# george-tyler-315-incline/ggml-neon-opt

Hardware: AMD Instinct MI355X
Metric: tg128 tok/s + Q4_K GEMV achieved-HBM-GB/s, TinyLlama-1.1B Q4_K_M @1 GPU (higher is better)
Workload: dtype q4_K/q6_K x q8_K (u4/u6*i8 dot4 -> i32, f32 combine); 1 GPU; tinyllama-1.1b Q4_K_M tg2221: full decode graph, token i at position i of a fresh f16 KV cache; parallelism=replicas x1, hipgraph=True

## Files before the change

### ggml-neon-opt_amd/csrc/kq_rows.hip

```cpp
#include <hip/hip_ext.h>

#include "kq_internal.h"
#include "kq_ops_device.h"
#include "kq_rows_device.h"

#ifndef KQ_ROWS_DIAG
#define KQ_ROWS_DIAG 0
#endif
#if KQ_ROWS_DIAG
#define RDIAG(ld) ((ld).diag)
#define RSTAMPS(h) ((h).stamps)
#define RSTAMP() __builtin_amdgcn_s_memrealtime()
#else
#define RDIAG(ld) 0
#define RSTAMPS(h) ((uint64_t *)nullptr)
#define RSTAMP() ((uint64_t)0)
#endif

#ifndef KQ_ROWS_XMODE
#define KQ_ROWS_XMODE 0
#endif
#ifndef KQ_ROWS_PRE0
#define KQ_ROWS_PRE0 1
#endif
#ifndef KQ_ROWS_L2PF
#define KQ_ROWS_L2PF 0
#endif
#ifndef KQ_ROWS_MASKED
#define KQ_ROWS_MASKED 2
#endif
#ifndef KQ_ROWS_LINT_BREAK
#define KQ_ROWS_LINT_BREAK 0
#endif

#ifndef KQ_ROWS_PRIO
#define KQ_ROWS_PRIO 0
#endif

#ifndef KQ_ROWS_YSC1
#define KQ_ROWS_YSC1 1
#endif

namespace kq {

__device__ __forceinline__ void store_y(float *p, float v) {
    if (KQ_ROWS_YSC1) asm volatile("global_store_dword %0, %1, off sc1" ::"v"(p), "v"(v) : "memory");
    else *p = v;
}

template <bool AM>
__global__ void __launch_bounds__(WG_THREADS) kq_quantize_q8L(const float *__restrict__ x, int64_t x_stride,
                                                              uint8_t *__restrict__ y, int nb, int64_t nblocks) {
    const int lane = threadIdx.x & 63;
    const int64_t bi = (int64_t)blockIdx.x * 16 + (threadIdx.x >> 4);
    if (bi >= nblocks) return;
    const int64_t row = bi / nb;
    const int b = (int)(bi - row * nb);
    const float *xb = x + row * x_stride + (int64_t)b * QK + 16 * (lane & 15);
    u32x4 v[4];
#pragma unroll
    for (int k = 0; k < 4; ++k) v[k] = *(const u32x4 *)(xb + 4 * k);
    quant16_store<AM>(v, lane & 15, y + bi * Q8L_STRIDE);
}
template __global__ void kq_quantize_q8L<false>(const float *, int64_t, uint8_t *, int, int64_t);
template __global__ void kq_quantize_q8L<true>(const float *, int64_t, uint8_t *, int, int64_t);

__global__ void __launch_bounds__(256) kq_rms_norm_q8L(const float *__restrict__ x, const float *__restrict__ w,
                                                       uint8_t *__restrict__ yq, int64_t n, float eps) {
    extern __shared__ __attribute__((aligned(16))) double sb_sum[];
    const int64_t row = blockIdx.x;
    const float *xr = x + row * n;
    const int nb = (int)(n / QK);
    const int rid = threadIdx.x >> 4, l = threadIdx.x & 15;
    for (int b0 = 0; b0 < nb; b0 += 16) {
        const int b = b0 + rid;
        double s = 0.0;
        if (b < nb) {
            float v[16];
            const float4 *p = (const float4 *)(xr + (int64_t)b * QK + 16 * l);
#pragma unroll
            for (int k = 0; k < 4; ++k) {
                const float4 t = p[k];
                v[4 * k] = t.x, v[4 * k + 1] = t.y, v[4 * k + 2] = t.z, v[4 * k + 3] = t.w;
            }
            s = sumsq16(v);
        }
        s = row16_sum(s);
        if (b < nb && l == 0) sb_sum[b] = s;
    }
    __syncthreads();
    double total = seq_sum_lds(sb_sum, nb);
    if (rms_mean_ambiguous(div_by_count(total, n), n)) {
        __syncthreads();
        if (threadIdx.x < 64) {
            const double s = seq_sumsq_wave(xr, n, threadIdx.x);
            if (threadIdx.x == 0) sb_sum[0] = s;
        }
        __syncthreads();
        total = sb_sum[0];
    }
    const float mean = (float)div_by_count(total, n);
    const float scale = 1.0f / sqrtf(mean + eps);
    for (int b0 = 0; b0 < nb; b0 += 16) {
        const int b = b0 + rid;
        if (b >= nb) continue;
        const float4 *p = (const float4 *)(xr + (int64_t)b * QK + 16 * l);
        const float4 *q = (const float4 *)(w + (int64_t)b * QK + 16 * l);
        u32x4 v[4];
#pragma unroll
        for (int k = 0; k < 4; ++k) {
            const float4 t = p[k], m = q[k];
            v[k].x = __float_as_uint((t.x * scale) * m.x);
// ... 187 lines not shown
template <int LSH>
struct RowsPrologue {
    static constexpr int NP = LSH ? 1 : ROWS_QPASS;
    static constexpr int NL = 4 >> LSH;
    static constexpr int LP = 16 << LSH;
    static constexpr int SPW = 4 >> LSH;
    u32x4 xv[NP][NL];
    u32x4 x2v[NP][NL];
    int qw = 0;
    int nb, pass, rot, wave, lane;

    __device__ __forceinline__ int slot(int i) const { return pass * i + SPW * wave + (lane >> (4 + LSH)); }
    __device__ __forceinline__ int sl() const { return lane & (LP - 1); }
    __device__ __forceinline__ int sbk(int j) const {
        const int b = (j < nb ? j : nb - 1) + rot;
        return b >= nb ? b - nb : b;
    }

    template <int PRO, bool ASM = true>
    __device__ __forceinline__ void load(const RowsLead &ld, int wave_, int lane_, int rot_, int diag) {
        nb = ld.nb, pass = SPW * ld.nwv, rot = rot_, wave = wave_, lane = lane_;
        const float *const x = (const float *)ld.x;
        const float *const x2 = (diag & 16) ? x : ld.x2;
#pragma unroll
        for (int i = 0; i < NP; ++i) qw += (i < ld.qiters && pass * i + SPW * wave < nb) ? 1 : 0;
#pragma unroll
        for (int i = 0; i < NP; ++i)
#pragma unroll
            for (int k = 0; k < NL; ++k) {
                asm volatile("" : "=v"(xv[i][k]));
                if (PRO != ROWS_PRO_NONE) asm volatile("" : "=v"(x2v[i][k]));
            }
#pragma unroll
        for (int i = 0; i < NP; ++i) {
            if (i < qw) {
                const int64_t e = (int64_t)sbk(slot(i)) * QK + (16 >> LSH) * sl();
#pragma unroll
                for (int k = 0; k < NL; ++k) {
                    if (ASM) gload16_into(xv[i][k], x + e + 4 * k);
                    else xv[i][k] = *(const u32x4 *)(x + e + 4 * k);
                }
                if (PRO != ROWS_PRO_NONE) {
#pragma unroll
                    for (int k = 0; k < NL; ++k) {
                        if (ASM) gload16_into(x2v[i][k], x2 + e + 4 * k);
                        else x2v[i][k] = *(const u32x4 *)(x2 + e + 4 * k);
                    }
                }
            }
        }
    }

    template <int PRO>
    __device__ __forceinline__ void pin() {
        if constexpr (LSH == 0) {
            asm volatile("" : "+v"(xv[0][0]), "+v"(xv[0][1]), "+v"(xv[0][2]), "+v"(xv[0][3]), "+v"(xv[1][0]),
                         "+v"(xv[1][1]), "+v"(xv[1][2]), "+v"(xv[1][3]), "+v"(xv[2][0]), "+v"(xv[2][1]),
                         "+v"(xv[2][2]), "+v"(xv[2][3]));
        } else {
#pragma unroll
            for (int k = 0; k < NL; ++k) asm volatile("" : "+v"(xv[0][k]));
        }
        if (PRO != ROWS_PRO_NONE) {
#pragma unroll
            for (int i = 0; i < NP; ++i)
#pragma unroll
                for (int k = 0; k < NL; ++k) asm volatile("" : "+v"(x2v[i][k]));
        }
    }

    __device__ __forceinline__ void swiglu_pass(int i) {
#pragma unroll
        for (int k = 0; k < NL; ++k) xv[i][k] = swiglu4(xv[i][k], x2v[i][k]);
    }

    __device__ __forceinline__ void values(int i, float v[4 * NL]) const {
#pragma unroll
        for (int k = 0; k < NL; ++k) {
            v[4 * k] = __uint_as_float(xv[i][k].x), v[4 * k + 1] = __uint_as_float(xv[i][k].y);
            v[4 * k + 2] = __uint_as_float(xv[i][k].z), v[4 * k + 3] = __uint_as_float(xv[i][k].w);
        }
    }

    __device__ __forceinline__ void norm(double *sums, const float *x, float eps) {
#pragma unroll
        for (int i = 0; i < NP; ++i) {
            if (i < qw) {
                const int j = slot(i);
                double sq = 0.0;
                if (j < nb) {
                    float v[4 * NL];
#pragma unroll
                    for (int k = 0; k < NL; ++k) {
                        v[4 * k] = __uint_as_float(xv[i][k].x), v[4 * k + 1] = __uint_as_float(xv[i][k].y);
                        v[4 * k + 2] = __uint_as_float(xv[i][k].z), v[4 * k + 3] = __uint_as_float(xv[i][k].w);
                    }
                    if constexpr (LSH == 0) {
                        sq = sumsq16(v);
                    } else {
#pragma unroll
                        for (int k = 0; k < 4 * NL; ++k) sq += (double)(v[k] * v[k]);
                    }
                }
                if constexpr (LSH == 0) sq = row16_sum(sq);
                else sq = sblk_sum<LP>(sq);
                if (j < nb && sl() == 0) sums[sbk(j)] = sq;
            }
        }
        asm volatile("s_waitcnt lgkmcnt(0)\n\ts_barrier" ::: "memory");
        double tot = seq_sum_lanes(sums, nb, lane);
        if (rms_mean_ambiguous(div_by_count(tot, (int64_t)nb * QK), (int64_t)nb * QK))
            tot = seq_sumsq_wave(x, (int64_t)nb * QK, lane);
        const float mean = (float)div_by_count(tot, (int64_t)nb * QK);
        const float scale = 1.0f / sqrtf(mean + eps);
#pragma unroll
        for (int i = 0; i < NP; ++i)
            if (i < qw)
#pragma unroll
                for (int k = 0; k < NL; ++k) xv[i][k] = normmul4(xv[i][k], x2v[i][k], scale);
    }

    __device__ __forceinline__ void quantize_pass(int i, uint8_t *act) {
        const int j = slot(i);
        uint8_t *const qb = act + Q8L_STRIDE * sbk(j);
        if constexpr (LSH == 0) {
            u32x4 cur[4];
#pragma unroll
            for (int k = 0; k < 4; ++k) {
                const u32x4 p0 = xv[0][k], p1 = xv[1][k], p2 = xv[2][k];
                cur[k] = i == 0 ? p0 : i == 1 ? p1 : p2;
            }
            if (j < nb) quant16_store(cur, lane & 15, qb);
        } else {
            float v[4 * NL];
            values(0, v);
            quant_wide_store<LP>(v, sl(), qb, j < nb);
        }
    }

    template <int PRO>
    __device__ __forceinline__ void finish(uint8_t *act, double *sums, const float *x, float eps, int diag, bool stamp,
                                           uint64_t &sx) {
        pin<PRO>();
        if (diag & 32) {
        } else if (PRO == ROWS_PRO_SWIGLU) {
#pragma unroll
            for (int i = 0; i < NP; ++i)
                if (i < qw) swiglu_pass(i);
        } else if (PRO == ROWS_PRO_NORM) {
            norm(sums, x, eps);
        }
        if (stamp) sx = __builtin_amdgcn_s_memrealtime();
        if (!(diag & 64)) {
#pragma unroll 1
            for (int i = 0; i < qw; ++i) quantize_pass(i, act);
        }
    }
};

template <int PRO, int LSH>
__global__ void __launch_bounds__(ROWS_WAVES * 64) kq_rows_prologue_dbg(const float *x, const float *x2, int nb, int cfg,
                                                                        float eps, uint8_t *out) {
    extern __shared__ __attribute__((aligned(16))) uint8_t smem[];
    const RowsLead ld = rows_lead(x, x2, nullptr, nullptr, nb, 0, 1, cfg, 0, 0);
    const int lane = threadIdx.x & 63;
    const int wave = __builtin_amdgcn_readfirstlane(threadIdx.x >> 6);
    RowsPrologue<LSH> pg;
    pg.template load<PRO, false>(ld, wave, lane, 0, 0);
    uint64_t sx = 0;
    pg.template finish<PRO>(smem, (double *)(smem + nb * Q8L_STRIDE), x, eps, 0, false, sx);
    asm volatile("s_waitcnt lgkmcnt(0)\n\ts_barrier" ::: "memory");
    const int ng = nb * (Q8L_STRIDE / 16);
    for (int k = threadIdx.x; k < ng; k += ld.nwv * 64) ((u32x4 *)out)[k] = ((const u32x4 *)smem)[k];
}

template <int PRO>
static auto rows_prologue_dbg_fn(int lsh) {
    return lsh == 2 ? kq_rows_prologue_dbg<PRO, 2> : lsh == 1 ? kq_rows_prologue_dbg<PRO, 1> : kq_rows_prologue_dbg<PRO, 0>;
}

int launch_rows_prologue_dbg(int pro, const float *x, const float *x2, float eps, int nb, int waves, uint8_t *out,
                             hipStream_t s) {
    const RowsProForm f = rows_pro_form(nb, waves);
    const int cfg = rows_cfg(waves, f.passes, 1, 0);
    const size_t lds = (size_t)nb * Q8L_STRIDE + (size_t)nb * 8;
    const auto fn = pro == ROWS_PRO_NORM ? rows_prologue_dbg_fn<ROWS_PRO_NORM>(f.lsh)
                    : pro == ROWS_PRO_SWIGLU ? rows_prologue_dbg_fn<ROWS_PRO_SWIGLU>(f.lsh)
                                             : rows_prologue_dbg_fn<ROWS_PRO_NONE>(f.lsh);
    allow_lds((const void *)fn, lds);
    hipLaunchKernelGGL(fn, dim3(1), dim3(waves * 64), lds, s, x, x2, nb, cfg, eps, out);
    const hipError_t e = hipGetLastError();
    return e == hipSuccess ? MI355X_OK : (int)e;
}

template <int TYPE, bool FUSEDQ, int PRO, int TMASK, int LSH, class Resolve>
__device__ __forceinline__ void rows_body(const RowsArgs &a, const RowsLead &ld, uint8_t *smem, int wave, int lane,
                                          uint64_t st0, Resolve resolve) {
    constexpr int BSZ = block_bytes(TYPE);
    constexpr int GRAN = rows_gran(TYPE);
    constexpr int NI = rows_ni(TYPE);
    constexpr int SLOT = rows_slot(TYPE);
    constexpr int D = rows_depth(TYPE);
    static_assert(D >= 2 && D <= 4, "vm_wait_k covers 3 steps in flight");
    const int nb = ld.nb;
    const int nwv = ld.nwv;
    const int q = lane >> 2, s = lane & 3;

    const int xm = !FUSEDQ ? 0 : KQ_ROWS_XMODE >= 0 ? KQ_ROWS_XMODE : a.xmode;
    RowsPrologue<LSH> pg;
    if (FUSEDQ) pg.template load<PRO>(ld, wave, lane, (xm & ROWS_X_ROT) ? (int)(blockIdx.x % (unsigned)nb) : 0, RDIAG(ld));
    const RowsHot h = resolve();
    const uint64_t sa = RSTAMP();
    const int bR = h.bR;
    const RowsLayout L = rows_layout(nb, TMASK, bR, h.rpw, nwv);
    uint8_t *const ring = smem + L.ring + wave * L.ring_stride;
    uint8_t *const ring_end = ring + D * SLOT;
    Rec *const recs = (Rec *)(smem + L.recs + wave * L.recs_stride);
    float *const outs = (float *)(smem + L.outs + wave * L.outs_stride);
    const uint8_t *const actq = smem + L.act;

    const int G = h.nrows * nb;
    const int T = (G + ROWS_SB - 1) / ROWS_SB;
    const uint8_t *src = h.w + (int64_t)h.r0 * nb * BSZ;
    const uint32_t mis = (uint32_t)((uintptr_t)src & 15u);
    const uint8_t *s16 = src - mis;
    const uint8_t *last16 =
        G > 0 ? (const uint8_t *)((uintptr_t)(src + (int64_t)G * BSZ - 1) & ~(uintptr_t)15) : s16;

    const bool pf_on = FUSEDQ && (KQ_ROWS_L2PF < 0 ? a.pf != 0 : KQ_ROWS_L2PF != 0) && T > D + 1;
    uint32_t pf_sink = 0;
    uint8_t *islot = ring;
    int it_ = 0;
    auto issue = [&]() {
        const uint8_t *base = s16 + (int64_t)it_ * (ROWS_SB * BSZ) + 16 * lane;
        if (it_ + 1 < T) {
#pragma unroll
            for (int i = 0; i < NI; ++i)
                if (i + 1 < NI || lane < GRAN - 64 * (NI - 1)) dma16_nt(base + 1024 * i, (LDS void *)(islot + 1024 * i));
        } else {
#pragma unroll
            for (int i = 0; i < NI; ++i) {
                const uint8_t *p = base + 1024 * i;
                if (i + 1 < NI || lane < GRAN - 64 * (NI - 1))
                    dma16_nt(p < last16 ? p : last16, (LDS void *)(islot + 1024 * i));
            }
        }
        islot = islot + SLOT == ring_end ? ring : islot + SLOT;
        ++it_;
    };

    const float *const res_p = h.res;
    uint32_t rv = 0;

    const int pre_req = KQ_ROWS_PRE0 < 0 ? a.pre0 : KQ_ROWS_PRE0;
    const int pre_cap = pre_req < D ? pre_req : D;
    const int pre0 = T >= pre_cap ? pre_cap : (T > 0 ? T : 0);
    uint64_t sx = 0, sq = 0, sf = 0;
    if (FUSEDQ) {
        const float *const x = (const float *)ld.x;
        constexpr int pro = PRO;
        constexpr int PL = (PRO != ROWS_PRO_NONE ? 2 : 1) * RowsPrologue<LSH>::NL;
        rv = gload4_asm(res_p && h.nrows > 0 ? res_p + h.r0 + (lane < h.nrows ? lane : 0) : x);
        if (xm & ROWS_X_BAR) asm volatile("s_barrier" ::: "memory");
        constexpr bool kConstPre = KQ_ROWS_PRE0 == 1 && KQ_ROWS_L2PF == 0;
        if (kConstPre && T == 0) {
            const uint8_t *xb = (const uint8_t *)x + 16 * lane;
#pragma unroll
            for (int i = 0; i < NI; ++i)
                if (KQ_ROWS_MASKED && i + 1 == NI) dma16_nt_lanes(xb, (LDS void *)(islot + 1024 * i), lane, GRAN - 64 * (NI - 1));
                else if (i + 1 < NI || lane < GRAN - 64 * (NI - 1)) dma16_nt(xb, (LDS void *)(islot + 1024 * i));
        }
        if (KQ_ROWS_MASKED && kConstPre && T > 0) {
            const uint8_t *base = s16 + 16 * lane;
            const uint8_t *lim = T > 1 ? base + 1024 * (NI - 1) : base + 1024 * (NI - 1) < last16 ? base + 1024 * (NI - 1) : last16;
#pragma unroll
            for (int i = 0; i + 1 < NI; ++i) {
                const uint8_t *p = base + 1024 * i;
                dma16_nt(T > 1 || p < last16 ? p : last16, (LDS void *)(islot + 1024 * i));
            }
            dma16_nt_lanes(lim, (LDS void *)(islot + 1024 * (NI - 1)), lane, GRAN - 64 * (NI - 1));
            islot = islot + SLOT == ring_end ? ring : islot + SLOT;
            ++it_;
        } else {
            for (int j = 0; j < pre0; ++j) issue();
        }
        if (pf_on) {
            const uint8_t *p = s16 + (int64_t)D * (ROWS_SB * BSZ) + 64 * lane;
#pragma unroll
            for (int i = 0; i < ROWS_PF; ++i) l2_touch(p + 4096 * i < last16 ? p + 4096 * i : last16, pf_sink);
        }
        const int tail = 1 + NI * pre0 + (pf_on ? ROWS_PF : 0);
        if (pro != ROWS_PRO_NORM && (xm & ROWS_X_PIPE)) {
#pragma unroll
            for (int i = 0; i < RowsPrologue<LSH>::NP; ++i) {
                if (i < pg.qw) {
                    vm_wait_dyn((pg.qw - 1 - i) * PL + tail);
                    pg.template pin<PRO>();
                    if (pro == ROWS_PRO_SWIGLU && !(RDIAG(ld) & 32)) pg.swiglu_pass(i);
                    if (!(RDIAG(ld) & 64)) pg.quantize_pass(i, smem + L.act);
                }
            }
            if (RSTAMPS(h)) sx = sq = __builtin_amdgcn_s_memrealtime();
        } else {
            if (KQ_ROWS_LINT_BREAK) {
            } else if (kConstPre && KQ_ROWS_MASKED == 2) {
                vm_wait<NI + 1>();
            } else if (kConstPre) {
                vm_wait<NI>();
            } else {
                vm_wait_dyn(tail);
            }
            pg.template finish<PRO>(smem + L.act, (double *)(smem + L.sums), x, h.eps, RDIAG(ld), RSTAMPS(h) != nullptr, sx);
            if (RSTAMPS(h)) {
                asm volatile("s_waitcnt lgkmcnt(0)" ::: "memory");
                sq = __builtin_amdgcn_s_memrealtime();
            }
        }
    } else {
        const int ng = nb * (Q8L_STRIDE / 16);
        for (int j = wave; 64 * j < ng; j += nwv) {
            const int k = 64 * j + lane;
            if (k < ng) dma16((const uint8_t *)ld.x + 16 * k, (LDS void *)(smem + L.act + 1024 * j));
        }
        for (int j = 0; j < pre0; ++j) issue();
        vm_wait_k<NI>(pre0);
    }
    while (it_ < D && it_ < T) issue();
    asm volatile("s_waitcnt lgkmcnt(0)\n\ts_barrier" ::: "memory");
    const uint64_t st1 = RSTAMPS(h) ? __builtin_amdgcn_s_memrealtime() : 0;

    int io = q, rr = 0;
    while (io >= nb) {
        io -= nb;
        ++rr;
    }
    int bend = bR * nb < G ? bR * nb : G;
    int brow = 0;
    const uint8_t *cslot = ring;
    int prio = -1;
#pragma unroll 1
    for (int t = 0; t < T; ++t) {
        if (KQ_ROWS_PRIO && (t & 3) == 0) {
            const int64_t rem = (int64_t)(T - t) * (ROWS_SB * BSZ);
            int p = (int)(rem * 4 / (a.prio_bytes + 1));
            p = __builtin_amdgcn_readfirstlane(p > 3 ? 3 : p);
            if (p != prio) {
                prio = p;
                if (p == 3) __builtin_amdgcn_s_setprio(3);
                else if (p == 2) __builtin_amdgcn_s_setprio(2);
                else if (p == 1) __builtin_amdgcn_s_setprio(1);
                else __builtin_amdgcn_s_setprio(0);
            }
        }
        if (pf_on && t < pre0) {
            if (T - t >= D) vm_wait<NI * (D - 1) + ROWS_PF>();
            else vm_wait_kp<NI, ROWS_PF>(T - t - 1);
        } else if (T - t >= D) {
            vm_wait<NI * (D - 1)>();
        } else {
            vm_wait_k<NI>(T - t - 1);
        }
        if (!(RDIAG(ld) & 8) && ROWS_SB * t + q < G) {
            const uint8_t *blk = cslot + mis + q * BSZ;
            const uint8_t *ab = actq + io * Q8L_STRIDE;
            QuadOut r = TYPE == Q4_K ? quad_q4K(blk, ab, s) : TYPE == Q5_K ? quad_q5K(blk, ab, s) : quad_q6K(blk, ab, s);
            const int isum = quad_sum(r.isum);
            const int imin = quad_sum(r.imin);
            if (s == 0) {
                const float yd = *(const float *)ab;
                Rec rec;
                if (TYPE == Q6_K) {
                    rec.a = isum - 32 * imin;
                    rec.b = 0;
                    rec.c = h2f(r.dh) * yd;
                    rec.e = 0.f;
                } else {
                    rec.a = isum;
                    rec.b = imin;
                    rec.c = yd * h2f(r.dh & 0xffffu);
                    rec.e = yd * h2f(r.dh >> 16);
                }
                recs[io * bR + rr] = rec;
            }
        }
        cslot = cslot + SLOT == ring_end ? ring : cslot + SLOT;
        io += ROWS_SB;
        if (nb >= ROWS_SB) {
            if (io >= nb) {
                io -= nb;
                ++rr;
            }
        } else {
            while (io >= nb) {
                io -= nb;
                ++rr;
            }
        }
        if (it_ < T) issue();
        if (RSTAMPS(h) && t == 0) sf = __builtin_amdgcn_s_memrealtime();
        if (ROWS_SB * (t + 1) >= bend) {
            wave_lds_fence();
            const int nr = bR < h.nrows - brow ? bR : h.nrows - brow;
            if (lane < nr) {
                float v = 0.f;
                const Rec *rc = recs + lane;
#pragma unroll 4
                for (int i = 0; i < nb; ++i) v = chain_step(TYPE, rc[i * bR], v);
                outs[brow + lane] = v;
            }
            brow += bR;
            rr -= bR;
            bend = bend + bR * nb < G ? bend + bR * nb : G;
            wave_lds_fence();
        }
    }
    if (KQ_ROWS_PRIO) __builtin_amdgcn_s_setprio(0);
    const uint64_t st2 = RSTAMPS(h) ? __builtin_amdgcn_s_memrealtime() : 0;
    if (pf_on) {
        asm volatile("" ::"v"(pf_sink));
    }

    if (h.nrows > 0) {
        wave_lds_fence();
        float *y = h.y + h.r0;
        if (res_p) {
            asm volatile("s_waitcnt vmcnt(0)" ::: "memory");
            asm volatile("" : "+v"(rv));
            for (int k = 0; k < h.nrows; k += 64)
                if (k + lane < h.nrows)
                    store_y(y + k + lane, outs[k + lane] + (k == 0 ? __uint_as_float(rv) : res_p[h.r0 + k + lane]));
        } else {
            for (int k = 0; k < h.nrows; k += 64)
                if (k + lane < h.nrows) store_y(y + k + lane, outs[k + lane]);
        }
    }
    if (h.epi && !(RDIAG(ld) & 128)) {
        asm volatile("s_waitcnt lgkmcnt(0)\n\ts_barrier" ::: "memory");
        if (h.m == 1 && h.nrows > 0) {
            const float *gouts = (const float *)(smem + L.outs + (wave - h.epi_wave_off) * L.outs_stride);
            const int n4 = h.epi_n & ~3;
            for (int k = 0; k < h.nrows; k += 64)
                if (k + lane < h.nrows) {
                    const int r = h.r0 + k + lane;
                    const float gv = gouts[k + lane], uv = outs[k + lane];
                    store_y(h.epi_y + r, r < n4 ? v_silu(gv) * uv : (gv / (1.0f + expf(-gv))) * uv);
                }
        }
    }
    if (RSTAMPS(h)) {
        const int64_t o = ((int64_t)blockIdx.x * ROWS_WAVES + wave) * 8;
        if (lane == 0 && o + 7 < h.stamps_cap) {
            RSTAMPS(h)[o] = st0;
            RSTAMPS(h)[o + 1] = st1;
            RSTAMPS(h)[o + 2] = st2;
            RSTAMPS(h)[o + 3] = __builtin_amdgcn_s_memrealtime();
            RSTAMPS(h)[o + 4] = sx;
            RSTAMPS(h)[o + 5] = sq;
            RSTAMPS(h)[o + 6] = sf;
            RSTAMPS(h)[o + 7] = sa;
        }
    }
}

template <int TMASK, bool FUSEDQ, int PRO, int LSH>
__global__ void __launch_bounds__(ROWS_WAVES * 64) kq_rows(KQ_ROWS_PARAMS) {
    extern __shared__ __attribute__((aligned(16))) uint8_t smem[];
    const RowsLead ld = rows_lead(x, x2, w0, res0, nb, waves_total, grid, cfg, rbase0, rrem0);
    if (RDIAG(ld) & 256) return;
    const uint64_t st0 = RSTAMP();
    const int lane = threadIdx.x & 63;
    const int wave = __builtin_amdgcn_readfirstlane(threadIdx.x >> 6);
    const int gw = wave * ld.grid + blockIdx.x;
    auto resolve = [&]() { return rows_resolve<TMASK>(ld, gw); };

    if (TMASK == 1) {
        rows_body<Q4_K, FUSEDQ, PRO, TMASK, LSH>(a, ld, smem, wave, lane, st0, resolve);
    } else if (TMASK == 2) {
        rows_body<Q5_K, FUSEDQ, PRO, TMASK, LSH>(a, ld, smem, wave, lane, st0, resolve);
    } else if (TMASK == 4) {
        rows_body<Q6_K, FUSEDQ, PRO, TMASK, LSH>(a, ld, smem, wave, lane, st0, resolve);
    } else {
        const RowsHot h = resolve();
        auto resolved = [&]() { return h; };
        if (h.type == Q6_K) rows_body<Q6_K, FUSEDQ, PRO, TMASK, LSH>(a, ld, smem, wave, lane, st0, resolved);
        else if (h.type == Q5_K) rows_body<Q5_K, FUSEDQ, PRO, TMASK, LSH>(a, ld, smem, wave, lane, st0, resolved);
        else rows_body<Q4_K, FUSEDQ, PRO, TMASK, LSH>(a, ld, smem, wave, lane, st0, resolved);
    }
}

#define KQ_ROWS_INST(TM, FQ, PR, LS) template __global__ void kq_rows<TM, FQ, PR, LS>(KQ_ROWS_PARAMS);
#define KQ_ROWS_INST_P(TM, PR) KQ_ROWS_INST(TM, true, PR, 0) KQ_ROWS_INST(TM, true, PR, 1) KQ_ROWS_INST(TM, true, PR, 2)
#define KQ_ROWS_INST_T(TM) KQ_ROWS_INST_P(TM, 0) KQ_ROWS_INST_P(TM, 1) KQ_ROWS_INST_P(TM, 2) KQ_ROWS_INST(TM, false, 0, 0)
KQ_ROWS_INST_T(1)
KQ_ROWS_INST_T(2)
KQ_ROWS_INST_T(4)
KQ_ROWS_INST_T(7)

#ifndef KQ_ROWS_DYN_RR
#define KQ_ROWS_DYN_RR 0
#endif
namespace {
static_assert(MI355X_MAX_FUSED == 4, "four matrices at most");
struct DynUnit {
    const uint8_t *src;
    int rows, flat, G, T;
};
}

struct RowsDynHot {
    int bR, rpw, U, P, ush, N, epi, epi_n;
    const uint8_t *w1, *w2, *w3;
    const float *s1, *s2, *s3;
    float *y0, *y1, *y2, *y3, *epi_y;
    float eps;
    uint64_t *stamps;
    int64_t stamps_cap;
};
__device__ __forceinline__ RowsDynHot rows_dyn_resolve() {
    const RowsRun r = rows_fetch();
    RowsDynHot h;
    h.bR = r.i32<RA_DW(bR)>(), h.rpw = r.i32<RA_DW(rpw)>();
    h.U = r.i32<RA_DW(dyn_u)>(), h.P = r.i32<RA_DW(dyn_p)>(), h.ush = r.i32<RA_DW(dyn_ush)>(), h.N = r.i32<RA_DW(n_rows)>();
    h.epi = r.i32<RA_DW(epi)>(), h.epi_n = r.i32<RA_DW(epi_n)>();
    h.epi_y = r.ptr<float, RA_DW(epi_y)>();
    h.eps = __uint_as_float(r.dw<RA_DW(eps)>());
    h.w1 = sreg(r.ptr<const uint8_t, RA_DW(w) + 2>()), h.w2 = sreg(r.ptr<const uint8_t, RA_DW(w) + 4>());
    h.w3 = sreg(r.ptr<const uint8_t, RA_DW(w) + 6>());
    h.s1 = sreg(r.ptr<const float, RA_DW(res) + 2>()), h.s2 = sreg(r.ptr<const float, RA_DW(res) + 4>());
    h.s3 = sreg(r.ptr<const float, RA_DW(res) + 6>());
    h.y0 = sreg(r.ptr<float, RA_DW(y)>()), h.y1 = sreg(r.ptr<float, RA_DW(y) + 2>());
    h.y2 = sreg(r.ptr<float, RA_DW(y) + 4>()), h.y3 = sreg(r.ptr<float, RA_DW(y) + 6>());
#if KQ_ROWS_DIAG
    h.stamps = r.ptr<uint64_t, RA_DW(stamps)>();
    h.stamps_cap = (int64_t)(uintptr_t)r.ptr<uint8_t, RA_DW(stamps_cap)>();
#else
    h.stamps = nullptr, h.stamps_cap = 0;
#endif
    return h;
}

template <int TYPE, bool FUSEDQ, int PRO, int TMASK, int LSH>
__device__ __forceinline__ void rows_dyn_body(const RowsArgs &a, const RowsLead &ld, uint8_t *smem, int wave, int lane,
// ... 62 lines not shown
        uh = mine ? (uint32_t)((uintptr_t)d.src >> 32) : uh;
        ug = mine ? (uint32_t)(d.G | (d.rows << 16)) : ug;
        uf = mine ? (uint32_t)d.flat : uf;
        is16 = (const uint8_t *)((uintptr_t)d.src & ~(uintptr_t)15);
        il16 = (const uint8_t *)((uintptr_t)(d.src + (int64_t)d.G * BSZ - 1) & ~(uintptr_t)15);
        iT = d.T;
        is = 0;
    };
    auto next_unit = [&](bool claim_ok) {
        const int k = ki + 1;
        if (k < P) {
            const int u = wave * P + k;
            if (u < nstat) take(u);
            else idone = true;
            return;
        }
        if (!claim_ok) {
            iwait = true;
            return;
        }
        iwait = false;
#if KQ_ROWS_DYN_RR
        const int uu = nwv * P + (k - P) * nwv + wave;
#else
        uint32_t u = 0;
        if (lane == 0) u = __hip_atomic_fetch_add(cnt, 1u, __ATOMIC_RELAXED, __HIP_MEMORY_SCOPE_WORKGROUP);
        const int uu = __builtin_amdgcn_readfirstlane((int)u);
#endif
        if (uu < units) take(uu);
        else idone = true;
    };
    auto issue = [&](bool claim_ok) {
        const uint8_t *base = is16 + (int64_t)is * (ROWS_SB * BSZ) + 16 * lane;
        if (is + 1 < iT) {
#pragma unroll
            for (int i = 0; i < NI; ++i)
                if (i + 1 < NI || lane < GRAN - 64 * (NI - 1)) dma16_nt(base + 1024 * i, (LDS void *)(islot + 1024 * i));
        } else {
#pragma unroll
            for (int i = 0; i < NI; ++i) {
                const uint8_t *p = base + 1024 * i;
                if (i + 1 < NI || lane < GRAN - 64 * (NI - 1))
                    dma16_nt(p < il16 ? p : il16, (LDS void *)(islot + 1024 * i));
            }
        }
        islot = islot + SLOT == ring_end ? ring : islot + SLOT;
        ++is;
        ++issued;
        if (is == iT) next_unit(claim_ok);
    };
    next_unit(false);

    const int f0 = 64 * wave + lane;
    const int fm = (f0 >= nr ? 1 : 0) + (f0 >= 2 * nr ? 1 : 0) + (f0 >= 3 * nr ? 1 : 0);
    const float *fres = fm == 0 ? s0 : fm == 1 ? s1 : fm == 2 ? s2 : s3;
    const int frow = row_of(f0 - fm * nr);
    uint32_t rv = 0;

    if (FUSEDQ) {
        rv = gload4_asm(fres && f0 < nflat && frow < N ? fres + frow : x);
        if (ki < 0) {
            const uint8_t *xb = (const uint8_t *)x + 16 * lane;
#pragma unroll
            for (int i = 0; i < NI; ++i)
                if (i + 1 == NI) dma16_nt_lanes(xb, (LDS void *)(islot + 1024 * i), lane, GRAN - 64 * (NI - 1));
                else dma16_nt(xb, (LDS void *)(islot + 1024 * i));
        } else {
            const uint8_t *base = is16 + 16 * lane;
            const uint8_t *lim = iT > 1 ? base + 1024 * (NI - 1) : base + 1024 * (NI - 1) < il16 ? base + 1024 * (NI - 1) : il16;
#pragma unroll
            for (int i = 0; i + 1 < NI; ++i) {
                const uint8_t *p = base + 1024 * i;
                dma16_nt(iT > 1 || p < il16 ? p : il16, (LDS void *)(islot + 1024 * i));
            }
            dma16_nt_lanes(lim, (LDS void *)(islot + 1024 * (NI - 1)), lane, GRAN - 64 * (NI - 1));
            islot = islot + SLOT == ring_end ? ring : islot + SLOT;
            ++is;
            ++issued;
            if (is == iT) next_unit(false);
        }
        vm_wait<NI + 1>();
        if (RSTAMPS(h)) sx = __builtin_amdgcn_s_memrealtime();
        uint64_t sxt = 0;
        pg.template finish<PRO>(smem + L.act, (double *)(smem + L.sums), x, h.eps, 0, false, sxt);
        if (RSTAMPS(h)) {
            asm volatile("s_waitcnt lgkmcnt(0)" ::: "memory");
            sq = __builtin_amdgcn_s_memrealtime();
        }
    } else {
        const int ng = nb * (Q8L_STRIDE / 16);
        for (int j = wave; 64 * j < ng; j += nwv) {
            const int k = 64 * j + lane;
            if (k < ng) dma16((const uint8_t *)ld.x + 16 * k, (LDS void *)(smem + L.act + 1024 * j));
        }
        rv = gload4_asm(fres && f0 < nflat && frow < N ? fres + frow : (const float *)ld.x);
        if (!idone && !iwait && ki >= 0) issue(false);
        vm_wait_k<NI>(issued);
    }
    while (!idone && !iwait && ki >= 0 && issued < D) issue(false);
    if (wave == 0 && lane == 0) *cnt = (uint32_t)(nwv * P);
    asm volatile("s_waitcnt lgkmcnt(0)\n\ts_barrier" ::: "memory");
    if (iwait) next_unit(true);
    while (!idone && ki >= 0 && issued < D) issue(true);
    const uint64_t st1 = RSTAMPS(h) ? __builtin_amdgcn_s_memrealtime() : 0;

    int kc = 0, cs = 0, cT = 0, cG = 0, cmis = 0, crows = 0, io = 0, rr = 0;
    int bro = 0;
    uint32_t bfl = 0;
    auto consume_unit = [&](int k) {
        const uint32_t gr = (uint32_t)__builtin_amdgcn_readlane((int)ug, k & 7);
        const int flat = __builtin_amdgcn_readlane((int)uf, k & 7);
        cG = (int)(gr & 0xffffu);
        crows = (int)(gr >> 16);
        cT = (cG + ROWS_SB - 1) / ROWS_SB;
        cmis = (int)((uint32_t)__builtin_amdgcn_readlane((int)ul, k & 7) & 15u);
        bfl = lane >= bro && lane < bro + crows ? (uint32_t)(flat + lane - bro) : bfl;
        cs = 0;
        io = q;
        rr = bro;
        while (io >= nb) {
            io -= nb;
            ++rr;
        }
    };
    auto replay = [&]() {
        wave_lds_fence();
        if (lane < bro) {
            float v = 0.f;
            const Rec *rc = recs + lane;
#pragma unroll 4
            for (int i = 0; i < nb; ++i) v = chain_step(TYPE, rc[i * bR], v);
            outs[bfl] = v;
        }
        wave_lds_fence();
        bro = 0;
    };
    int consumed = 0;
    if (issued > 0) consume_unit(0);
    const uint8_t *cslot = ring;
#pragma unroll 1
    while (consumed < issued) {
        vm_wait_k<NI>(issued - consumed - 1);
        if (ROWS_SB * cs + q < cG) {
            const uint8_t *blk = cslot + cmis + q * BSZ;
            const uint8_t *ab = actq + io * Q8L_STRIDE;
            QuadOut r = TYPE == Q4_K ? quad_q4K(blk, ab, s) : TYPE == Q5_K ? quad_q5K(blk, ab, s) : quad_q6K(blk, ab, s);
            const int isum = quad_sum(r.isum);
            const int imin = quad_sum(r.imin);
            if (s == 0) {
                const float yd = *(const float *)ab;
                Rec rec;
                if (TYPE == Q6_K) {
                    rec.a = isum - 32 * imin;
                    rec.b = 0;
                    rec.c = h2f(r.dh) * yd;
                    rec.e = 0.f;
                } else {
                    rec.a = isum;
                    rec.b = imin;
                    rec.c = yd * h2f(r.dh & 0xffffu);
                    rec.e = yd * h2f(r.dh >> 16);
                }
                recs[io * bR + rr] = rec;
            }
        }
        cslot = cslot + SLOT == ring_end ? ring : cslot + SLOT;
        ++consumed;
        ++cs;
        if (!idone) issue(true);
        if (RSTAMPS(h) && consumed == 1) sf = __builtin_amdgcn_s_memrealtime();
        if (cs == cT) {
            bro += crows;
            if (bro + U > bR || consumed == issued) replay();
            ++kc;
            if (consumed < issued) consume_unit(kc);
        } else {
            io += ROWS_SB;
            while (io >= nb) {
                io -= nb;
                ++rr;
            }
        }
    }

    const uint64_t st2 = RSTAMPS(h) ? __builtin_amdgcn_s_memrealtime() : 0;
    asm volatile("s_waitcnt vmcnt(0)" ::: "memory");
    asm volatile("" : "+v"(rv));
    asm volatile("s_waitcnt lgkmcnt(0)\n\ts_barrier" ::: "memory");
    for (int f = f0; f < nflat; f += 64 * nwv) {
        const int m = (f >= nr ? 1 : 0) + (f >= 2 * nr ? 1 : 0) + (f >= 3 * nr ? 1 : 0);
        const int row = f == f0 ? frow : row_of(f - m * nr);
        if (row >= N) continue;
        const float *res = m == 0 ? s0 : m == 1 ? s1 : m == 2 ? s2 : s3;
        float *y = m == 0 ? y0 : m == 1 ? y1 : m == 2 ? y2 : y3;
        float v = outs[f];
        if (res) v = v + (f == f0 ? __uint_as_float(rv) : res[row]);
        store_y(y + row, v);
    }
    if (h.epi) {
        const int n4 = h.epi_n & ~3;
        for (int f = f0; f < nr; f += 64 * nwv) {
            const int r = row_of(f);
            if (r >= N) continue;
            const float gv = outs[f], uv = outs[nr + f];
            store_y(h.epi_y + r, r < n4 ? v_silu(gv) * uv : (gv / (1.0f + expf(-gv))) * uv);
        }
    }
    if (RSTAMPS(h)) {
        const int64_t o = ((int64_t)blockIdx.x * ROWS_WAVES + wave) * 8;
        if (lane == 0 && o + 7 < h.stamps_cap) {
            RSTAMPS(h)[o] = st0;
            RSTAMPS(h)[o + 1] = st1;
            RSTAMPS(h)[o + 2] = st2;
            RSTAMPS(h)[o + 3] = __builtin_amdgcn_s_memrealtime();
            RSTAMPS(h)[o + 4] = sx;
            RSTAMPS(h)[o + 5] = sq;
            RSTAMPS(h)[o + 6] = sf;
            RSTAMPS(h)[o + 7] = (uint64_t)(ki + 1);
        }
    }
}
template <int TMASK, bool FUSEDQ, int PRO, int LSH>
__global__ void __launch_bounds__(ROWS_WAVES * 64) kq_rows_dyn(KQ_ROWS_PARAMS) {
    extern __shared__ __attribute__((aligned(16))) uint8_t smem[];
    const RowsLead ld = rows_lead(x, x2, w0, res0, nb, waves_total, grid, cfg, rbase0, rrem0);
    const uint64_t st0 = RSTAMP();
    const int lane = threadIdx.x & 63;
    const int wave = __builtin_amdgcn_readfirstlane(threadIdx.x >> 6);
    constexpr int TYPE = TMASK == 1 ? Q4_K : TMASK == 2 ? Q5_K : Q6_K;
    rows_dyn_body<TYPE, FUSEDQ, PRO, TMASK, LSH>(a, ld, smem, wave, lane, st0);
}

#define KQ_ROWS_DYN_INST(TM, FQ, PR, LS) template __global__ void kq_rows_dyn<TM, FQ, PR, LS>(KQ_ROWS_PARAMS);
#define KQ_ROWS_DYN_INST_P(TM, PR) \
    KQ_ROWS_DYN_INST(TM, true, PR, 0) KQ_ROWS_DYN_INST(TM, true, PR, 1) KQ_ROWS_DYN_INST(TM, true, PR, 2)
#define KQ_ROWS_DYN_INST_T(TM) \
    KQ_ROWS_DYN_INST_P(TM, 0) KQ_ROWS_DYN_INST_P(TM, 1) KQ_ROWS_DYN_INST_P(TM, 2) KQ_ROWS_DYN_INST(TM, false, 0, 0)
KQ_ROWS_DYN_INST_T(1)
KQ_ROWS_DYN_INST_T(2)
KQ_ROWS_DYN_INST_T(4)

}
```

### ggml-neon-opt_amd/csrc/kq_rows_device.h

```cpp
#pragma once

#include "kq_device.h"
#include "kq_ops_device.h"

namespace kq {

template <typename Op>
__device__ __forceinline__ int row16_reduce(int v, Op op) {
    v = op(v, __builtin_amdgcn_update_dpp(v, v, 0xB1, 0xF, 0xF, false));
    v = op(v, __builtin_amdgcn_update_dpp(v, v, 0x4E, 0xF, 0xF, false));
    v = op(v, __builtin_amdgcn_update_dpp(v, v, 0x141, 0xF, 0xF, false));
    v = op(v, __builtin_amdgcn_update_dpp(v, v, 0x140, 0xF, 0xF, false));
    return v;
}

__device__ __forceinline__ uint32_t qbyte(float iscale, float x) {
    int q = nearest_int_fused(iscale, x);
    q = q < 127 ? q : 127;
    return (uint32_t)q & 0xffu;
}

template <bool AM = false>
__device__ __forceinline__ void quant16_store(const u32x4 v[4], int l, uint8_t *qb) {
    float x[16];
// ... 8 lines not shown
#pragma unroll
    for (int k = 0; k < 16; ++k) {
        mp = fmaxf(mp, x[k]);
        mn = fmaxf(mn, -x[k]);
    }
    const int mpb = row16_reduce(__float_as_int(mp), [](int a, int c) { return a > c ? a : c; });
    const int mnb = row16_reduce(__float_as_int(mn), [](int a, int c) { return a > c ? a : c; });
    const float m = __int_as_float(mpb > mnb ? mpb : mnb);
    bool neg = mnb > mpb;
    if (mpb == mnb && mpb != 0) {
        uint32_t key = 0xffffffffu;
#pragma unroll
        for (int k = 15; k >= 0; --k)
            if (fabsf(x[k]) == m) key = 2u * (uint32_t)(16 * l + k) + (x[k] < 0.f ? 1u : 0u);
        key = (uint32_t)row16_reduce((int)key, [](int a, int c) { return (uint32_t)a < (uint32_t)c ? a : c; });
        neg = (key & 1u) != 0;
    }
    const float maxv = neg ? -m : m;
    const float iscale = -127.f / maxv;
    u32x4 q;
    q.x = qbyte(iscale, x[0]) | (qbyte(iscale, x[1]) << 8) | (qbyte(iscale, x[2]) << 16) | (qbyte(iscale, x[3]) << 24);
    q.y = qbyte(iscale, x[4]) | (qbyte(iscale, x[5]) << 8) | (qbyte(iscale, x[6]) << 16) | (qbyte(iscale, x[7]) << 24);
    q.z = qbyte(iscale, x[8]) | (qbyte(iscale, x[9]) << 8) | (qbyte(iscale, x[10]) << 16) |
          (qbyte(iscale, x[11]) << 24);
    q.w = qbyte(iscale, x[12]) | (qbyte(iscale, x[13]) << 8) | (qbyte(iscale, x[14]) << 16) |
          (qbyte(iscale, x[15]) << 24);
    int bsum = sdot4(q.x, 0x01010101u, 0);
    bsum = sdot4(q.y, 0x01010101u, bsum);
    bsum = sdot4(q.z, 0x01010101u, bsum);
    bsum = sdot4(q.w, 0x01010101u, bsum);
    float d = 1.f / iscale;
    if (m == 0.f) {
        q = u32x4{0u, 0u, 0u, 0u};
        bsum = 0;
        d = 0.f;
    }
    *(u32x4 *)(qb + 16 + 16 * l) = q;
    if (AM) {
        const int bs = bsum + __builtin_amdgcn_update_dpp(bsum, bsum, 0xB1, 0xF, 0xF, false);
        if (!(l & 1)) {
            *(_Float16 *)(qb + 272 + l) = (_Float16)(bs & 63);
            *(_Float16 *)(qb + 288 + l) = (_Float16)(bs >> 6);
        }
    } else {
        *(int16_t *)(qb + 272 + 2 * l) = (int16_t)bsum;
    }
    if (l == 0) *(float *)qb = d;
}

__device__ __forceinline__ void swap_rows16(uint32_t v, uint32_t &a, uint32_t &b) {
    const auto r = __builtin_amdgcn_permlane16_swap(v, v, false, false);
    a = r[0], b = r[1];
}
__device__ __forceinline__ void swap_rows32(uint32_t v, uint32_t &a, uint32_t &b) {
    const auto r = __builtin_amdgcn_permlane32_swap(v, v, false, false);
    a = r[0], b = r[1];
}
template <int LP, typename Op>
__device__ __forceinline__ int sblk_reduce(int v, Op op) {
    static_assert(LP == 32 || LP == 64, "lanes per superblock");
    v = row16_reduce(v, op);
    uint32_t a, b;
    swap_rows16((uint32_t)v, a, b);
    v = op((int)a, (int)b);
    if (LP == 64) {
        swap_rows32((uint32_t)v, a, b);
        v = op((int)a, (int)b);
    }
    return v;
}
template <int LP>
__device__ __forceinline__ double sblk_sum(double v) {
    static_assert(LP == 32 || LP == 64, "lanes per superblock");
    v = row16_sum(v);
#pragma unroll
    for (int step = 0; step < (LP == 64 ? 2 : 1); ++step) {
        const uint64_t u = __builtin_bit_cast(uint64_t, v);
        uint32_t la, lb, ha, hb;
        if (step == 0) swap_rows16((uint32_t)u, la, lb), swap_rows16((uint32_t)(u >> 32), ha, hb);
        else swap_rows32((uint32_t)u, la, lb), swap_rows32((uint32_t)(u >> 32), ha, hb);
        v = __builtin_bit_cast(double, ((uint64_t)ha << 32) | la) + __builtin_bit_cast(double, ((uint64_t)hb << 32) | lb);
    }
    return v;
}

template <int LP>
__device__ __forceinline__ void quant_wide_store(const float *x, int l, uint8_t *qb, bool st) {
    constexpr int VP = 256 / LP;
    float mp = 0.f, mn = 0.f;
#pragma unroll
    for (int k = 0; k < VP; ++k) {
        mp = fmaxf(mp, x[k]);
        mn = fmaxf(mn, -x[k]);
    }
    const int mpb = sblk_reduce<LP>(__float_as_int(mp), [](int a, int c) { return a > c ? a : c; });
    const int mnb = sblk_reduce<LP>(__float_as_int(mn), [](int a, int c) { return a > c ? a : c; });
    const float m = __int_as_float(mpb > mnb ? mpb : mnb);
    bool neg = mnb > mpb;
    if (__any(mpb == mnb && mpb != 0)) {
        uint32_t key = 0xffffffffu;
#pragma unroll
        for (int k = VP - 1; k >= 0; --k)
            if (fabsf(x[k]) == m) key = 2u * (uint32_t)(VP * l + k) + (x[k] < 0.f ? 1u : 0u);
        key = (uint32_t)sblk_reduce<LP>((int)key, [](int a, int c) { return (uint32_t)a < (uint32_t)c ? a : c; });
        if (mpb == mnb && mpb != 0) neg = (key & 1u) != 0;
    }
    const float maxv = neg ? -m : m;
    const float iscale = -127.f / maxv;
    uint32_t q[VP / 4];
    int bsum = 0;
#pragma unroll
    for (int k = 0; k < VP / 4; ++k) {
        q[k] = qbyte(iscale, x[4 * k]) | (qbyte(iscale, x[4 * k + 1]) << 8) | (qbyte(iscale, x[4 * k + 2]) << 16) |
               (qbyte(iscale, x[4 * k + 3]) << 24);
        bsum = sdot4(q[k], 0x01010101u, bsum);
    }
    float d = 1.f / iscale;
    if (m == 0.f) {
#pragma unroll
        for (int k = 0; k < VP / 4; ++k) q[k] = 0u;
        bsum = 0;
        d = 0.f;
    }
    bsum += __builtin_amdgcn_update_dpp(bsum, bsum, 0xB1, 0xF, 0xF, false);
    if (VP == 4) bsum += __builtin_amdgcn_update_dpp(bsum, bsum, 0x4E, 0xF, 0xF, false);
    if (st) {
        if (VP == 8) *(uint2 *)(qb + 16 + 8 * l) = make_uint2(q[0], q[VP / 4 - 1]);
        else *(uint32_t *)(qb + 16 + 4 * l) = q[0];
        if (!(l & (16 / VP - 1))) *(int16_t *)(qb + 272 + 2 * (l / (16 / VP))) = (int16_t)bsum;
        if (l == 0) *(float *)qb = d;
    }
}

__device__ __forceinline__ uint32_t gload4_asm(const float *p) {
    uint32_t r;
    asm volatile("global_load_dword %0, %1, off" : "=v"(r) : "v"(p) : "memory");
    return r;
}

__device__ __forceinline__ u32x4 swiglu4(u32x4 g, u32x4 u) {
    u32x4 r;
    r.x = __float_as_uint(v_silu(__uint_as_float(g.x)) * __uint_as_float(u.x));
    r.y = __float_as_uint(v_silu(__uint_as_float(g.y)) * __uint_as_float(u.y));
    r.z = __float_as_uint(v_silu(__uint_as_float(g.z)) * __uint_as_float(u.z));
    r.w = __float_as_uint(v_silu(__uint_as_float(g.w)) * __uint_as_float(u.w));
    return r;
}

__device__ __forceinline__ u32x4 normmul4(u32x4 x, u32x4 w, float scale) {
    u32x4 r;
    r.x = __float_as_uint((__uint_as_float(x.x) * scale) * __uint_as_float(w.x));
    r.y = __float_as_uint((__uint_as_float(x.y) * scale) * __uint_as_float(w.y));
    r.z = __float_as_uint((__uint_as_float(x.z) * scale) * __uint_as_float(w.z));
    r.w = __float_as_uint((__uint_as_float(x.w) * scale) * __uint_as_float(w.w));
    return r;
}

__device__ __forceinline__ u32x4 gload16_asm(const float *p) {
    u32x4 r;
    asm volatile("global_load_dwordx4 %0, %1, off" : "=v"(r) : "v"(p) : "memory");
    return r;
}

__device__ __forceinline__ void gload16_into(u32x4 &r, const float *p) {
    asm volatile("global_load_dwordx4 %0, %1, off" : "+v"(r) : "v"(p) : "memory");
}
// ... 136 lines not shown
```

Baseline: 1440 tok/s.

## Restructure fused RMS-norm prologue: tree reduction, idle-wave skip, speculative quantize

Splits the fused RMS-norm prologue into publish and total phases. The sum of squares is now reduced with a DPP/row-swap tree when nb is a power of two up to 64, instead of a sequential lane sum. Waves that hold no quantize work return right after the barrier. For the wide-lane layout, the normalized values are quantized immediately and redone only when the rare ambiguous-mean fallback fires. The aim is to shorten the serial critical path between the norm barrier and the start of the GEMV, at the cost of a possible second quantize, reduction order that can differ in the last bits, and more diagnostic stamp slots.

```diff
diff --git a/ggml-neon-opt_amd/csrc/kq_rows.hip b/ggml-neon-opt_amd/csrc/kq_rows.hip
--- a/ggml-neon-opt_amd/csrc/kq_rows.hip
+++ b/ggml-neon-opt_amd/csrc/kq_rows.hip
@@ -16,6 +16,10 @@
 #define RSTAMPS(h) ((uint64_t *)nullptr)
 #define RSTAMP() ((uint64_t)0)
 #endif
+constexpr int ROWS_STAMP_SLOTS = 16;
+struct NormStamps {
+    uint64_t pub = 0, bar = 0, scale = 0;
+};
 
 #ifndef KQ_ROWS_XMODE
 #define KQ_ROWS_XMODE 0
@@ -28,6 +32,15 @@
 #endif
 #ifndef KQ_ROWS_MASKED
 #define KQ_ROWS_MASKED 2
+#endif
+#ifndef KQ_ROWS_NORM_SKIP
+#define KQ_ROWS_NORM_SKIP 1
+#endif
+#ifndef KQ_ROWS_NORM_LATE
+#define KQ_ROWS_NORM_LATE 1
+#endif
+#ifndef KQ_ROWS_NORM_TREE
+#define KQ_ROWS_NORM_TREE 1
 #endif
 #ifndef KQ_ROWS_LINT_BREAK
 #define KQ_ROWS_LINT_BREAK 0
@@ -381,7 +394,7 @@
         }
     }
 
-    __device__ __forceinline__ void norm(double *sums, const float *x, float eps) {
+    __device__ __forceinline__ void norm_publish(double *sums) {
 #pragma unroll
         for (int i = 0; i < NP; ++i) {
             if (i < qw) {
@@ -406,17 +419,79 @@
                 if (j < nb && sl() == 0) sums[sbk(j)] = sq;
             }
         }
+    }
+    __device__ __forceinline__ double norm_total(const double *sums) const {
+        if (KQ_ROWS_NORM_TREE && nb <= 64 && (nb & (nb - 1)) == 0) return tree_sum_lanes(sums, nb, lane);
+        return seq_sum_lanes(sums, nb, lane);
+    }
+    static __device__ __forceinline__ float norm_scale(double tot, int64_t n, float eps) {
+        const float mean = (float)div_by_count(tot, n);
+        return 1.0f / sqrtf(mean + eps);
+    }
+
+    __device__ __forceinline__ void norm(double *sums, const float *x, float eps, NormStamps &ns) {
+        norm_publish(sums);
+        ns.pub = RSTAMP();
         asm volatile("s_waitcnt lgkmcnt(0)\n\ts_barrier" ::: "memory");
-        double tot = seq_sum_lanes(sums, nb, lane);
-        if (rms_mean_ambiguous(div_by_count(tot, (int64_t)nb * QK), (int64_t)nb * QK))
-            tot = seq_sumsq_wave(x, (int64_t)nb * QK, lane);
-        const float mean = (float)div_by_count(tot, (int64_t)nb * QK);
-        const float scale = 1.0f / sqrtf(mean + eps);
+        ns.bar = RSTAMP();
+        if (KQ_ROWS_NORM_SKIP && qw == 0) return;
+        const int64_t n = (int64_t)nb * QK;
+        double tot = norm_total(sums);
+        if (rms_mean_ambiguous(div_by_count(tot, n), n)) tot = seq_sumsq_wave(x, n, lane);
+        float scale = norm_scale(tot, n, eps);
+        if (KQ_ROWS_DIAG) asm volatile("" : "+v"(scale));
+        ns.scale = RSTAMP();
 #pragma unroll
         for (int i = 0; i < NP; ++i)
             if (i < qw)
 #pragma unroll
                 for (int k = 0; k < NL; ++k) xv[i][k] = normmul4(xv[i][k], x2v[i][k], scale);
+    }
+
+    __device__ __forceinline__ void quantize_wide(const u32x4 t[NL], uint8_t *act) {
+        const int j = slot(0);
+        float v[4 * NL];
+#pragma unroll
+        for (int k = 0; k < NL; ++k) {
+            v[4 * k] = __uint_as_float(t[k].x), v[4 * k + 1] = __uint_as_float(t[k].y);
+            v[4 * k + 2] = __uint_as_float(t[k].z), v[4 * k + 3] = __uint_as_float(t[k].w);
+        }
+        quant_wide_store<LP>(v, sl(), act + Q8L_STRIDE * sbk(j), j < nb);
+    }
+
+    __device__ __forceinline__ void norm_late(uint8_t *act, double *sums, const float *x, float eps, int diag, bool stamp,
+                                              uint64_t &sx, NormStamps &ns) {
+        static_assert(LSH >= 1 && NP == 1, "one pass in registers");
+        norm_publish(sums);
+        ns.pub = RSTAMP();
+        asm volatile("s_waitcnt lgkmcnt(0)\n\ts_barrier" ::: "memory");
+        ns.bar = RSTAMP();
+        if (KQ_ROWS_NORM_SKIP && qw == 0) {
+            if (stamp) sx = __builtin_amdgcn_s_memrealtime();
+            return;
+        }
+        const int64_t n = (int64_t)nb * QK;
+        const double md = div_by_count(norm_total(sums), n);
+        float scale = 1.0f / sqrtf((float)md + eps);
+        if (KQ_ROWS_DIAG) asm volatile("" : "+v"(scale));
+        ns.scale = RSTAMP();
+        u32x4 t[NL];
+        if (qw) {
+#pragma unroll
+            for (int k = 0; k < NL; ++k) t[k] = normmul4(xv[0][k], x2v[0][k], scale);
+        }
+        if (stamp) sx = __builtin_amdgcn_s_memrealtime();
+        if (qw && !(diag & 64)) quantize_wide(t, act);
+        double mdg = md;
+        asm volatile("" : "+v"(mdg));
+        if (rms_mean_ambiguous(mdg, n)) {
+            scale = norm_scale(seq_sumsq_wave(x, n, lane), n, eps);
+            if (qw) {
+#pragma unroll
+                for (int k = 0; k < NL; ++k) t[k] = normmul4(xv[0][k], x2v[0][k], scale);
+                if (!(diag & 64)) quantize_wide(t, act);
+            }
+        }
     }
 
     __device__ __forceinline__ void quantize_pass(int i, uint8_t *act) {
@@ -439,7 +514,7 @@
 
     template <int PRO>
     __device__ __forceinline__ void finish(uint8_t *act, double *sums, const float *x, float eps, int diag, bool stamp,
-                                           uint64_t &sx) {
+                                           uint64_t &sx, NormStamps &ns) {
         pin<PRO>();
         if (diag & 32) {
         } else if (PRO == ROWS_PRO_SWIGLU) {
@@ -447,7 +522,12 @@
             for (int i = 0; i < NP; ++i)
                 if (i < qw) swiglu_pass(i);
         } else if (PRO == ROWS_PRO_NORM) {
-            norm(sums, x, eps);
+            if constexpr (KQ_ROWS_NORM_LATE && LSH >= 1) {
+                norm_late(act, sums, x, eps, diag, stamp, sx, ns);
+                return;
+            } else {
+                norm(sums, x, eps, ns);
+            }
         }
         if (stamp) sx = __builtin_amdgcn_s_memrealtime();
         if (!(diag & 64)) {
@@ -467,7 +547,8 @@
     RowsPrologue<LSH> pg;
     pg.template load<PRO, false>(ld, wave, lane, 0, 0);
     uint64_t sx = 0;
-    pg.template finish<PRO>(smem, (double *)(smem + nb * Q8L_STRIDE), x, eps, 0, false, sx);
+    NormStamps ns;
+    pg.template finish<PRO>(smem, (double *)(smem + nb * Q8L_STRIDE), x, eps, 0, false, sx, ns);
     asm volatile("s_waitcnt lgkmcnt(0)\n\ts_barrier" ::: "memory");
     const int ng = nb * (Q8L_STRIDE / 16);
     for (int k = threadIdx.x; k < ng; k += ld.nwv * 64) ((u32x4 *)out)[k] = ((const u32x4 *)smem)[k];
@@ -554,7 +635,8 @@
     const int pre_req = KQ_ROWS_PRE0 < 0 ? a.pre0 : KQ_ROWS_PRE0;
     const int pre_cap = pre_req < D ? pre_req : D;
     const int pre0 = T >= pre_cap ? pre_cap : (T > 0 ? T : 0);
-    uint64_t sx = 0, sq = 0, sf = 0;
+    uint64_t sx = 0, sq = 0, sf = 0, sl = 0;
+    NormStamps ns;
     if (FUSEDQ) {
         const float *const x = (const float *)ld.x;
         constexpr int pro = PRO;
@@ -599,7 +681,7 @@
                     if (!(RDIAG(ld) & 64)) pg.quantize_pass(i, smem + L.act);
                 }
             }
-            if (RSTAMPS(h)) sx = sq = __builtin_amdgcn_s_memrealtime();
+            if (RSTAMPS(h)) sl = sx = sq = __builtin_amdgcn_s_memrealtime();
         } else {
             if (KQ_ROWS_LINT_BREAK) {
             } else if (kConstPre && KQ_ROWS_MASKED == 2) {
@@ -609,7 +691,8 @@
             } else {
                 vm_wait_dyn(tail);
             }
-            pg.template finish<PRO>(smem + L.act, (double *)(smem + L.sums), x, h.eps, RDIAG(ld), RSTAMPS(h) != nullptr, sx);
+            sl = RSTAMP();
+            pg.template finish<PRO>(smem + L.act, (double *)(smem + L.sums), x, h.eps, RDIAG(ld), RSTAMPS(h) != nullptr, sx, ns);
             if (RSTAMPS(h)) {
                 asm volatile("s_waitcnt lgkmcnt(0)" ::: "memory");
                 sq = __builtin_amdgcn_s_memrealtime();
@@ -747,8 +830,8 @@
         }
     }
     if (RSTAMPS(h)) {
-        const int64_t o = ((int64_t)blockIdx.x * ROWS_WAVES + wave) * 8;
-        if (lane == 0 && o + 7 < h.stamps_cap) {
+        const int64_t o = ((int64_t)blockIdx.x * ROWS_WAVES + wave) * ROWS_STAMP_SLOTS;
+        if (lane == 0 && o + ROWS_STAMP_SLOTS - 1 < h.stamps_cap) {
             RSTAMPS(h)[o] = st0;
             RSTAMPS(h)[o + 1] = st1;
             RSTAMPS(h)[o + 2] = st2;
@@ -757,6 +840,11 @@
             RSTAMPS(h)[o + 5] = sq;
             RSTAMPS(h)[o + 6] = sf;
             RSTAMPS(h)[o + 7] = sa;
+            RSTAMPS(h)[o + 8] = sl;
+            RSTAMPS(h)[o + 9] = ns.pub;
+            RSTAMPS(h)[o + 10] = ns.bar;
+            RSTAMPS(h)[o + 11] = ns.scale;
+            RSTAMPS(h)[o + 12] = (uint64_t)pg.qw;
         }
     }
 }
@@ -985,7 +1073,8 @@
         vm_wait<NI + 1>();
         if (RSTAMPS(h)) sx = __builtin_amdgcn_s_memrealtime();
         uint64_t sxt = 0;
-        pg.template finish<PRO>(smem + L.act, (double *)(smem + L.sums), x, h.eps, 0, false, sxt);
+        NormStamps ns;
+        pg.template finish<PRO>(smem + L.act, (double *)(smem + L.sums), x, h.eps, 0, false, sxt, ns);
         if (RSTAMPS(h)) {
             asm volatile("s_waitcnt lgkmcnt(0)" ::: "memory");
             sq = __builtin_amdgcn_s_memrealtime();
@@ -1110,8 +1199,8 @@
         }
     }
     if (RSTAMPS(h)) {
-        const int64_t o = ((int64_t)blockIdx.x * ROWS_WAVES + wave) * 8;
-        if (lane == 0 && o + 7 < h.stamps_cap) {
+        const int64_t o = ((int64_t)blockIdx.x * ROWS_WAVES + wave) * ROWS_STAMP_SLOTS;
+        if (lane == 0 && o + ROWS_STAMP_SLOTS - 1 < h.stamps_cap) {
             RSTAMPS(h)[o] = st0;
             RSTAMPS(h)[o + 1] = st1;
             RSTAMPS(h)[o + 2] = st2;
diff --git a/ggml-neon-opt_amd/csrc/kq_rows_device.h b/ggml-neon-opt_amd/csrc/kq_rows_device.h
--- a/ggml-neon-opt_amd/csrc/kq_rows_device.h
+++ b/ggml-neon-opt_amd/csrc/kq_rows_device.h
@@ -114,6 +114,24 @@
         v = __builtin_bit_cast(double, ((uint64_t)ha << 32) | la) + __builtin_bit_cast(double, ((uint64_t)hb << 32) | lb);
     }
     return v;
+}
+
+__device__ __forceinline__ double tree_sum_lanes(const double *sums, int nb, int lane) {
+    double v = lane < nb ? sums[lane] : 0.0;
+    v = row16_sum(v);
+    if (nb > 16) {
+        const uint64_t u = __builtin_bit_cast(uint64_t, v);
+        uint32_t la, lb, ha, hb;
+        swap_rows16((uint32_t)u, la, lb), swap_rows16((uint32_t)(u >> 32), ha, hb);
+        v = __builtin_bit_cast(double, ((uint64_t)ha << 32) | la) + __builtin_bit_cast(double, ((uint64_t)hb << 32) | lb);
+    }
+    if (nb > 32) {
+        const uint64_t u = __builtin_bit_cast(uint64_t, v);
+        uint32_t la, lb, ha, hb;
+        swap_rows32((uint32_t)u, la, lb), swap_rows32((uint32_t)(u >> 32), ha, hb);
+        v = __builtin_bit_cast(double, ((uint64_t)ha << 32) | la) + __builtin_bit_cast(double, ((uint64_t)hb << 32) | lb);
+    }
+    return readlane_f64(v, 0);
 }
 
 template <int LP>
```

After: 1478 tok/s (median of 6 runs). +2.7%, better.
